# osqp/miosqp

Hardware: AMD Instinct MI355X
Metric: ADMM iterations/s (random_miqp n=500 m=1000 p=250, node-at-a-time B&B) (higher is better)
Workload: dtype f64

## Files before the change

### include/miosqp_amd.h

```cpp
#ifndef MIOSQP_AMD_H
#define MIOSQP_AMD_H

#include <stdint.h>

#ifdef __cplusplus
extern "C" {
#endif

#define MIOSQP_QP_SOLVED 1
#define MIOSQP_QP_MAX_ITER_REACHED (-2)
#define MIOSQP_QP_PRIMAL_INFEASIBLE (-3)
#define MIOSQP_QP_DUAL_INFEASIBLE (-4)
#define MIOSQP_QP_UNSOLVED (-10)

#define MIOSQP_EARG (-1)
#define MIOSQP_EHIP (-2)
#define MIOSQP_EFACTOR (-3)
#define MIOSQP_ENODEV (-4)
#define MIOSQP_EUNSUPPORTED (-5)
#define MIOSQP_EFULL (-6)
#define MIOSQP_EBOUNDS 1

typedef struct miosqp_qp_settings {
  double rho;
// ... 288 lines not shown
  int32_t improved;
  int32_t reserved;
  double upper_glob, lower_glob;
  double device_time;
  double run_time;
} miosqp_search_info;

int miosqp_qp_search_create(miosqp_qp_engine *e, int32_t capacity);
int miosqp_qp_search_reset(miosqp_qp_engine *e);
int miosqp_qp_search_add_leaf(miosqp_qp_engine *e, const double *l_int, const double *u_int, const double *x0,
                              const double *y0, int32_t depth, double lower);
int miosqp_qp_search_take_leaf(miosqp_qp_engine *e, double *l_int, double *u_int, double *x0, double *y0,
                               int32_t *depth, double *lower);
int miosqp_qp_search_set_incumbent(miosqp_qp_engine *e, double upper, const double *x);
int miosqp_qp_search_get_incumbent(miosqp_qp_engine *e, double *upper, double *x);
int miosqp_qp_search_run(miosqp_qp_engine *e, int32_t tree_explor_rule, int64_t max_nodes, double budget_s,
                         miosqp_search_info *info);

typedef struct miosqp_pool_digest {
  int32_t slot;
  int32_t status_val;
  int32_t iter;
  int32_t int_inf;
  int32_t nextvar;
  int32_t reserved;
  double lower;
  double heur_viol;
  double heur_obj;
  double pri_res, dua_res;
} miosqp_pool_digest;
// ... 74 lines not shown
```

### miosqp_amd/_lib.py

```python
import ctypes as C
import os

_PKG = os.path.dirname(os.path.abspath(__file__))
LIB_PATH = os.path.join(_PKG, "libmiosqp_hip.so")

dp = C.POINTER(C.c_double)
ip = C.POINTER(C.c_int32)
i64p = C.POINTER(C.c_int64)


class Settings(C.Structure):
    _fields_ = [(k, C.c_double) for k in
                ("rho", "sigma", "alpha", "eps_abs", "eps_rel", "eps_prim_inf", "eps_dual_inf")] + \
               [(k, C.c_int32) for k in ("max_iter", "scaling", "check_termination", "warm_start",
                                         "device", "max_batch", "fold", "resident", "setup_on_device", "coop", "pers", "batch_pers",
                                         "rho_auto")]


class Info(C.Structure):
    _fields_ = [("status_val", C.c_int32), ("iter", C.c_int32), ("run_time", C.c_double),
                ("obj_val", C.c_double), ("pri_res", C.c_double), ("dua_res", C.c_double),
                ("device_time", C.c_double), ("lower", C.c_double),
                ("int_inf", C.c_int32), ("nextvar", C.c_int32), ("heur_viol", C.c_double),
                ("heur_obj", C.c_double)]
# ... 115 lines not shown
    "miosqp_qp_solve_trees_lockstep_sb": (C.c_int, [C.c_void_p, C.c_int32, dp, dp, dp, dp, dp, dp, dp, C.c_int32, C.c_int32,
                                                    C.c_int32, C.c_int32, C.c_int32, C.c_int32, C.c_int32, C.c_double, dp,
                                                    C.POINTER(TreeInfo), C.POINTER(LockstepStats),
                                                    C.POINTER(LockstepSbStats)]),
    "miosqp_qp_solve_trees_lockstep_ahead": (C.c_int, [C.c_void_p, C.c_int32, dp, dp, dp, dp, dp, dp, dp, C.c_int32,
                                                       C.c_int32, C.c_int32, C.c_int32, dp, C.POINTER(TreeInfo),
                                                       C.POINTER(LockstepStats), C.POINTER(LockstepAheadStats)]),
    "miosqp_qp_solve_trees_refill": (C.c_int, [C.c_void_p, C.c_int32, dp, dp, dp, dp, dp, dp, dp, C.c_int32, C.c_int32,
                                               C.c_int32, dp, C.POINTER(TreeInfo), C.POINTER(RefillStats)]),
    "miosqp_qp_search_create": (C.c_int, [C.c_void_p, C.c_int32]),
    "miosqp_qp_search_reset": (C.c_int, [C.c_void_p]),
    "miosqp_qp_search_add_leaf": (C.c_int, [C.c_void_p, dp, dp, dp, dp, C.c_int32, C.c_double]),
    "miosqp_qp_search_take_leaf": (C.c_int, [C.c_void_p, dp, dp, dp, dp, C.POINTER(C.c_int32), C.POINTER(C.c_double)]),
    "miosqp_qp_search_set_incumbent": (C.c_int, [C.c_void_p, C.c_double, dp]),
    "miosqp_qp_search_get_incumbent": (C.c_int, [C.c_void_p, C.POINTER(C.c_double), dp]),
    "miosqp_qp_search_run": (C.c_int, [C.c_void_p, C.c_int32, C.c_int64, C.c_double, C.POINTER(SearchInfo)]),
    "miosqp_qp_stream_create": (C.c_int, [C.c_void_p, C.c_int32, C.c_int32, C.c_int32]),
    "miosqp_qp_stream_begin": (C.c_int, [C.c_void_p]),
    "miosqp_qp_stream_add_leaf": (C.c_int, [C.c_void_p, dp, dp, dp, dp, C.c_int32, C.c_double]),
    "miosqp_qp_stream_take_leaf": (C.c_int, [C.c_void_p, dp, dp, dp, dp, C.POINTER(C.c_int32), C.POINTER(C.c_double)]),
    "miosqp_qp_stream_set_incumbent": (C.c_int, [C.c_void_p, C.c_double, dp]),
    "miosqp_qp_stream_get_incumbent": (C.c_int, [C.c_void_p, C.POINTER(C.c_double), dp]),
    "miosqp_qp_stream_step": (C.c_int, [C.c_void_p, C.c_int32, C.c_int32, C.c_int32, C.c_int64, C.POINTER(StreamInfo)]),
    "miosqp_qp_solve_batch": (C.c_int, [C.c_void_p, C.c_int32, dp, dp, dp, dp, dp, dp,
                                        C.POINTER(Info)]),
    "miosqp_qp_solve_batch_q": (C.c_int, [C.c_void_p, C.c_int32, dp, dp, dp, dp, dp, dp, dp,
                                          C.POINTER(Info)]),
    "miosqp_qp_solve_tree": (C.c_int, [C.c_void_p, dp, dp, dp, dp, C.c_double, dp, C.c_int32, C.c_int32, dp,
                                       C.POINTER(TreeInfo)]),
    "miosqp_qp_pool_create": (C.c_int, [C.c_void_p, C.c_int32, C.c_int32]),
# ... 70 lines not shown
```

### miosqp_amd/csrc/engine.hip

```cpp
#include <hip/hip_runtime.h>

#include <dlfcn.h>
#include <sys/stat.h>

#include <algorithm>
#include <chrono>
#include <cmath>
#include <cstdio>
#include <cstdlib>
#include <cstring>
#include <map>
#include <mutex>
#include <queue>
#include <deque>
#include <tuple>
#include <type_traits>
#include <string>
#include <vector>

#include "../../include/miosqp_amd.h"
#include "factor.hpp"
#include "polish_many.hpp"
#include "polish_many_large.hpp"
#include "lockstep_trees.hpp"
// ... 77 lines not shown
  int digest;
  int bm_ablate;
  unsigned long long *prof;
  const double *W;
  int ldw;
  unsigned *coop_tag;
  unsigned long long *coop_buf;
  unsigned long long *coop_chk;
  unsigned long long *coop_q;
  unsigned long long *coop_reg;
  unsigned long long *coop_chz;
  unsigned long long *coop_dec;
  int coop_nt;
  int coop_lag;
  int coop_tres;
  const double *Kc;
  int coop_dbg;
  int coop_nap;
  int coop_stride;
  size_t coop_half;
  const double *coop_W;
  int coop_ldw, coop_mg;
  const int *coop_brow;
  const double *coop_aj;
  int Bs;
  double *b_l, *b_u, *b_x, *b_z, *b_y, *b_wh, *b_rx, *b_cv, *b_ut, *b_xt, *b_dx, *b_dy;
  double *b_xfs;
  double *b_sm, *b_sn;
  double *b_xfin, *b_yfin;
  double *b_xi, *b_xis;
// ... 2244 lines not shown
    return pad;
  }
  if (which == 4) {
    ChipTurn *t = chip_of(e);
    if (!t) return -1;
    std::lock_guard<std::mutex> lk(t->mu);
    return t->users;
  }
  if (which == 5) return (e->pers_capable && e->pp.sinv && e->pp.res_w) ? e->n - e->pp.res_c0 : 0;
  if (which == 6) return (e->pers_capable && e->pp.sinv && e->pp.sym) ? e->pp.sym_tiles : 0;
  if (which == 7) return e->kbs_launches;
  if (which == 8) return e->kbs_chunks_run;
  if (which == 9) return e->graph_chunks_run;
  if (which == 10) return e->run_nap_in_use;
  if (which == 11) return e->run_cal_nodes;
  if (which == 12) return e->polml ? (int64_t)(e->polml->cap_slab * sizeof(double)) : 0;
  return which == 0 ? e->compactions : which == 1 ? e->kbp_fallbacks : -1;
}

int miosqp_qp_get_batch_stats(miosqp_qp_engine *e, double *ms, int64_t *batch_iters, int64_t *node_iters,
                              int32_t reset) {
  if (!e) return MIOSQP_EARG;
  if (ms) *ms = e->bloop_ms;
  if (batch_iters) *batch_iters = e->bloop_iters;
  if (node_iters) *node_iters = e->bloop_node_iters;
  if (reset) {
    e->bloop_ms = 0.0;
    e->bloop_iters = e->bloop_node_iters = 0;
  }
  return 0;
// ... 86 lines not shown
```

### miosqp_amd/csrc/host.inc

```
constexpr int POOL_EVENTS = 8;
constexpr int COOP_RETRY = -1000;

inline int pick_tpr(double avg_row) {
  if (avg_row <= 48) return 16;
  if (avg_row <= 192) return 32;
  if (avg_row <= 640) return 64;
  if (avg_row <= 1536) return 128;
  return 256;
}

#define DISPATCH_TPR(tpr, KERNEL, rows, stream, ...)                                              \
  do {                                                                                            \
    switch (tpr) {                                                                                \
      case 16: hipLaunchKernelGGL(KERNEL<16>, dim3(((rows) + 15) / 16), dim3(256), 0, stream, __VA_ARGS__); break;   \
      case 32: hipLaunchKernelGGL(KERNEL<32>, dim3(((rows) + 7) / 8), dim3(256), 0, stream, __VA_ARGS__); break;     \
      case 64: hipLaunchKernelGGL(KERNEL<64>, dim3(((rows) + 3) / 4), dim3(256), 0, stream, __VA_ARGS__); break;     \
      case 128: hipLaunchKernelGGL(KERNEL<128>, dim3(((rows) + 1) / 2), dim3(256), 0, stream, __VA_ARGS__); break;   \
      default: hipLaunchKernelGGL(KERNEL<256>, dim3(rows), dim3(256), 0, stream, __VA_ARGS__); break;                \
    }                                                                                             \
  } while (0)

std::mutex g_capture_mutex;

struct ParkedChunk {
// ... 411 lines not shown
  return 8;
}
int coop_pick_testers(int spare) {
  int nt = spare >= 8 ? std::min(COOP_NT_MAX, spare) : 0;
  if (const char *ev = getenv("MIOSQP_COOP_TESTERS")) nt = std::max(0, std::min(std::min(COOP_NT_MAX, spare), atoi(ev)));
  return nt;
}
void coop_pick_lag(miosqp_qp_engine *e) {
  Dev &d = e->d;
  const int n = e->n, M = e->M, N = n + M, nt = d.coop_nt;
  bool res = nt > 0 && (N % 2) == 0 && N - (M & ~1) <= 128 * COOP_RC_S && M <= COOP_RC_R * nt * 8 && n <= COOP_RV_R * nt * 8 &&
             N <= 128 * COOP_RV_S;
  if (const char *ev = getenv("MIOSQP_COOP_TRES")) res = res && atoi(ev) != 0;
  d.coop_tres = res ? 1 : 0;
  d.coop_lag = res ? 10 : 16;
  if (const char *ev = getenv("MIOSQP_COOP_LAG")) d.coop_lag = std::max(1, atoi(ev));
}

#define COOP_FORMS(X) \
  X(8, 2, 2) X(8, 2, 4) X(8, 3, 4) X(8, 4, 4)
int coop_occupancy(int rw, int cpt, int cptf) {
  int per_cu = 0;
  hipError_t oq = hipErrorInvalidValue;
#define X(RW, CPT, CPTF) \
  if (rw == RW && cpt == CPT && cptf == CPTF) oq = hipOccupancyMaxActiveBlocksPerMultiprocessor(&per_cu, k_coop<512, RW, CPT, CPTF, true>, 512, 0);
  COOP_FORMS(X)
#undef X
  return oq == hipSuccess ? per_cu : 0;
}

// ... 1155 lines not shown
```

### miosqp_amd/csrc/host_search.inc

```
namespace {

struct NodeSearch {
  int cap = 0;
  double *lo = nullptr, *hi = nullptr, *x = nullptr, *y = nullptr, *inc_x = nullptr;
  double *own_block = nullptr;
  SearchDigest *dg = nullptr;
  unsigned long long seq = 0;
  hipEvent_t ev[4] = {};
  int ev_slot = 0;
  bool ev_pending = false;
  unsigned long long *stamps = nullptr;
  std::vector<int> stamp_iter;
  CoopRun *run_blk = nullptr;
  CoopRun run_blk_host;
  bool run_blk_sent = false;
  unsigned long long *mail_host = nullptr, *mail_dev = nullptr;
  unsigned long long mtag = 0;
  bool run_live = false;
  hipEvent_t ev_run[2] = {};
  int64_t run_off = 0;
  int run_nap = -1;
  std::vector<int> open;
  std::vector<int> freelist, depth, parent, kids;
  std::vector<char> decided;
// ... 429 lines not shown
  S.upper = upper;
  S.have_inc = true;
  search_prune(S);
  return 0;
}

int miosqp_qp_search_get_incumbent(miosqp_qp_engine *e, double *upper, double *x) {
  if (!e || !e->search || !upper || !x) return MIOSQP_EARG;
  ENTER(e);
  NodeSearch &S = *search_of(e);
  *upper = S.upper;
  if (S.have_inc) {
    HIPCHK(hipMemcpyAsync(x, S.inc_x, sizeof(double) * e->n, hipMemcpyDeviceToHost, e->stream));
    HIPCHK(hipStreamSynchronize(e->stream));
  }
  return 0;
}

int miosqp_qp_search_run(miosqp_qp_engine *e, int32_t tree_explor_rule, int64_t max_nodes, double budget_s,
                         miosqp_search_info *info) {
  if (!e || !e->search || !info || tree_explor_rule < 0 || tree_explor_rule > 3) return MIOSQP_EARG;
  ENTER(e);
  NodeSearch &S = *search_of(e);
  const double t0 = wall();
  const size_t n = e->n, M = e->M, p = e->d.n_int;
  const Dev &d = e->d;
  int64_t done = 0, it_sum = 0;
  int improved = 0, rc_full = 0;
  double dev_ms = 0.0;
  if (int rc = run_end(e, S, true, nullptr, nullptr)) return rc;
// ... 157 lines not shown
      if (!g.pad) break;
      reset_registration(e);
      g_err = "cooperative solver: " + std::string(g.pad == 1 ? "the grid was not co-resident within 100 ms (device shared?)"
                                                               : "exchange timed out") + ", stage " + std::to_string(g.pad);
      if (g.pad != 1) return MIOSQP_EHIP;
      if (S.ev_pending) {
        HIPCHK(hipEventSynchronize(S.ev[2 * S.ev_slot + 1]));
        S.ev_pending = false;
      }
      e->loop_iters -= g.iter;
      if (!e->node_it.empty()) e->node_it.pop_back();
      int rc = leave_coop(e);
      if (rc) return rc;
    }
    if (S.stamps) S.stamp_iter[a.seq % 256] = g.todo ? -1 : g.iter;
    done++;
    S.nodes++;
    S.iters += g.iter;
    it_sum += g.iter;
    bool branch = false;
    const bool ok = g.status == MIOSQP_QP_SOLVED || g.status == MIOSQP_QP_MAX_ITER_REACHED;
    if (ok) {
      S.lower[s] = g.lower;
      if (!(g.lower > S.upper)) {
        if (g.int_inf == 0) {
          S.upper = g.lower;
          S.have_inc = true;
          improved = 1;
          search_prune(S);
        } else {
// ... 75 lines not shown
```

### miosqp_amd/csrc/kernels_coop.inc

```
constexpr unsigned long long COOP_LIMIT_REGISTER = 10000000ull, COOP_LIMIT_EXCHANGE = 200000000ull;
__device__ __forceinline__ bool coop_expired(unsigned &spins, unsigned long long &since,
                                             unsigned long long limit = COOP_LIMIT_EXCHANGE) {
  if ((++spins & 4095u) != 0u) return false;
  const unsigned long long now = wall_clock64();
  if (spins == 4096u) {
    since = now;
    return false;
  }
  return now - since > limit;
}

typedef unsigned ll_u4 __attribute__((ext_vector_type(4)));
__device__ __forceinline__ void ll_publish(unsigned long long *slot, double v, unsigned tag) {
  ll_u4 w;
  w.x = (unsigned)__double2loint(v); w.y = tag; w.z = (unsigned)__double2hiint(v); w.w = tag;
  asm volatile("global_store_dwordx4 %0, %1, off sc1\n\ts_nop 1" ::"v"(slot), "v"(w) : "memory");
}
__device__ __forceinline__ ll_u4 ll_peek(const unsigned long long *slot) {
  ll_u4 w;
  asm volatile("global_load_dwordx4 %0, %1, off sc1" : "=v"(w) : "v"(slot) : "memory");
  return w;
}

constexpr unsigned long long COOP_SENTINEL = 0x7FF0000000005EA7ull;
// ... 393 lines not shown
  return v;
}

struct CoopTesterArgs {
  unsigned long long *coop_chk, *coop_chz, *coop_q, *coop_dec, *prof;
  const double *Kc, *Einv, *E, *Dinv, *D, *l, *u, *q;
  Ctrl *ctrl;
  int n, M, ldw;
  double c, cinv, eps_abs, eps_rel, eps_pinf, eps_dinf;
  int epi;
  unsigned long long *stamps;
  int res;
  int run;
  unsigned long long *coop_buf, coop_half;
  int NR, lag;
};
#define COOP_STAMP(ptr, k)                                          \
  do {                                                              \
    if ((ptr) != nullptr && threadIdx.x == 0) (ptr)[k] = wall_clock64(); \
  } while (0)

__device__ __forceinline__ double coop_prow(const int *__restrict__ idx, const double *__restrict__ val, int s, int e, int t, int tpr,
                                            const lds_f64 *v) {
  double a0 = 0.0, a1 = 0.0;
  for (int k = s + 2 * t; k < e; k += 2 * tpr) {
    const double2 a = *reinterpret_cast<const double2 *>(val + k);
    const int2 j = *reinterpret_cast<const int2 *>(idx + k);
    a0 = fma(a.x, v[j.x], a0);
    a1 = fma(a.y, v[j.y], a1);
  }
  return a0 + a1;
// ... 86 lines not shown
  const CoopEpi &d = *dp;
  const int t = threadIdx.x, n = d.n, M = d.M;
  lds_f64 *const ox = to_lds(s1), *const xi = to_lds(s1) + 1024, *const xis = to_lds(s2);
  const lds_f64 *const lx = to_lds(lv0);
  for (int i = t; i < n; i += COOP_B) {
    double o = d.D[i] * lx[M + i];
    const int k = d.int_pos[i];
    if (k >= 0) o = fmin(fmax(o, epi_ld(d.a.lo_s + k, d.coh)), epi_ld(d.a.hi_s + k, d.coh));
    ox[i] = o;
    const double r = k >= 0 ? rint(o) : o;
    xi[i] = r;
    xis[i] = d.Dinv[i] * r;
  }
  __syncthreads();
  COOP_STAMP(stamps, 11);
  double vmax = -1.7e308;
  const int Gh = COOP_B / d.tpr_h, Go = COOP_B / d.tpr_o;
  const int CH = (M + Gh - 1) / Gh, CO = (n + Go - 1) / Go;
  for (int c = w; c < CH + CO; c += G) {
    if (c < CH) {
      const int tpr = d.tpr_h, g = t / tpr, tr = t % tpr;
      const int row_raw = c * Gh + g;
      const bool live = row_raw < M;
      const int row = live ? row_raw : M - 1;
      const double ei = d.Einv[row], rl = d.root_l[row], ru = d.root_u[row];
      double acc[1];
      acc[0] = coop_prow(d.pc_idx, d.pc_A, d.pc_ptr[row], d.pc_ptr[row + 1], tr, tpr, xis);
      coop_row_reduce<1>(acc, tpr, red);
      if (live && tr == 0) {
        const double z = ei * acc[0];
// ... 17 lines not shown
  COOP_STAMP(stamps, 12);
  {
    for (int off = 32; off > 0; off >>= 1) vmax = fmax(vmax, __shfl_xor(vmax, off, 64));
    __syncthreads();
    if ((t & 63) == 0) red[t >> 6] = vmax;
    __syncthreads();
    if (t == 0) {
      double r = red[0];
      for (int k = 1; k < COOP_B / 64; k++) r = fmax(r, red[k]);
      ll_publish(d.epi_buf + 2 * (size_t)(2 * n + w), r, tag);
    }
    __syncthreads();
  }
}
template <int COOP_B>
__device__ __attribute__((noinline)) void coop_epi_commit(const CoopEpi *dp, unsigned long long *stamps, const int G, const unsigned tag,
                                                const int st, const int it, const double *lv0, double *s1, double *s2, double *red,
                                                const double *rec, int *s_fail) {
  const CoopEpi &d = *dp;
  const int t = threadIdx.x, n = d.n, M = d.M, p = d.n_int;
  lds_f64 *const ox = to_lds(s1), *const xi = to_lds(s1) + 1024;
  lds_f64 *const vals = to_lds(s2);
  const lds_f64 *const ly = to_lds(lv0);
  COOP_STAMP(stamps, 8);
  int cnt = 0, bestk = 0x7fffffff;
  double best = -1.0;
  for (int k = t; k < p; k += COOP_B) {
    const double v = ox[d.i_idx[k]], f = fabs(v - rint(v));
    cnt += f > d.eps_int;
    if (f > best) { best = f; bestk = k; }
  }
  for (int off = 32; off > 0; off >>= 1) {
    const double ob = __shfl_xor(best, off, 64);
// ... 3 lines not shown
  }
  __shared__ double sb[COOP_B / 64];
  __shared__ int sk[COOP_B / 64], sc[COOP_B / 64], s_dig[2];
  if ((t & 63) == 0) { sb[t >> 6] = best; sk[t >> 6] = bestk; sc[t >> 6] = cnt; }
  __syncthreads();
  if (t == 0) {
    for (int k = 1; k < COOP_B / 64; k++) {
      cnt += sc[k];
      if (sb[k] > best || (sb[k] == best && sk[k] < bestk)) { best = sb[k]; bestk = sk[k]; }
    }
    s_dig[0] = cnt;
    s_dig[1] = bestk == 0x7fffffff ? -1 : bestk;
  }
  __syncthreads();
  const int int_inf = s_dig[0], nv = s_dig[1];
  for (int i = t; i < n; i += COOP_B) epi_st(d.a.x_s + i, ox[i], d.coh);
  for (int r = t; r < M; r += COOP_B) epi_st(d.a.y_s + r, d.cinv * d.E[r] * ly[r], d.coh);
  {
    const int ne = 2 * n + G;
    constexpr int KE = (COOP_EPI_ENTRIES + COOP_B - 1) / COOP_B;
    bool have[KE];
#pragma unroll
    for (int k = 0; k < KE; k++) have[k] = t + k * COOP_B >= ne;
    unsigned spins = 0;
    unsigned long long since = 0;
    static_assert(KE == 5, "ll_peek_wait5");
    for (;;) {
      const unsigned long long *ptr[KE];
      ll_u4 w[KE];
#pragma unroll
      for (int k = 0; k < KE; k++) ptr[k] = d.epi_buf + (have[k] ? 0 : 2 * (size_t)(t + k * COOP_B));
      ll_peek_wait5(ptr, w);
      bool all = true;
#pragma unroll
      for (int k = 0; k < KE; k++) {
        if (have[k]) continue;
        if (w[k].y == tag && w[k].w == tag) {
          vals[t + k * COOP_B] = __hiloint2double((int)w[k].z, (int)w[k].x);
          have[k] = true;
        } else {
          all = false;
        }
      }
      if (__syncthreads_and(all)) break;
      if (coop_expired(spins, since)) {
        *s_fail = 1;
        d.ctrl->pad = 12;
      }
      if (__syncthreads_or(*s_fail)) break;
    }
  }
  __syncthreads();
  if (*s_fail) return;
  COOP_STAMP(stamps, 9);
  const double lower = coop_block_sum1024(vals, n, red);
  const double hobj = coop_block_sum1024(vals + n, n, red);
  __syncthreads();
  double hviol = -1.7e308;
  for (int k = t; k < G; k += COOP_B) hviol = fmax(hviol, vals[2 * n + k]);
  for (int off = 32; off > 0; off >>= 1) hviol = fmax(hviol, __shfl_xor(hviol, off, 64));
  if ((t & 63) == 0) red[t >> 6] = hviol;
  __syncthreads();
  hviol = red[0];
  for (int k = 1; k < COOP_B / 64; k++) hviol = fmax(hviol, red[k]);
  __syncthreads();
  COOP_STAMP(stamps, 14);
  int action = 0, branched = 0;
  if (!(lower > d.a.upper)) {
    if (int_inf == 0) {
      action = 1;
    } else {
      if (hviol <= 0.0 && hobj < d.a.upper) action = 2;
      if (nv >= 0) {
        branched = 1;
        const double xv = ox[d.i_idx[nv]];
        for (int q = t; q < p; q += COOP_B) {
          const double lo = epi_ld(d.a.lo_s + q, d.coh), hi = epi_ld(d.a.hi_s + q, d.coh);
          epi_st(d.a.lo0 + q, lo, d.coh);
          epi_st(d.a.hi0 + q, q == nv ? floor(xv) : hi, d.coh);
          epi_st(d.a.lo1 + q, q == nv ? ceil(xv) : lo, d.coh);
          epi_st(d.a.hi1 + q, hi, d.coh);
        }
      }
    }
  }
  if (action) {
    const lds_f64 *src = action == 1 ? ox : xi;
    for (int i = t; i < n; i += COOP_B) epi_st(d.a.inc_x + i, src[i], d.coh);
  }
  if (d.coh) {
    asm volatile("s_waitcnt vmcnt(0)" ::: "memory");
    __syncthreads();
  }
  COOP_STAMP(stamps, 15);
  if (t == 0) {
    Ctrl *c = d.ctrl;
    c->status = st;
    c->done = 1;
    c->int_inf = int_inf;
    c->nextvar = nv;
    c->lower = lower;
    c->heur_obj = hobj;
    c->heur_viol = hviol;
    const lds_f64 *const rc = to_lds(rec);
    coop_record(d.a.dg, st, it, int_inf, nv, action, branched, lower, hviol, hobj, rc[0], rc[1], rc[2], d.t_node, d.a.seq);
    COOP_STAMP(stamps, 10);
  }
}

constexpr int COOP_RC_R = 3, COOP_RC_S = 4, COOP_RV_R = 1, COOP_RV_S = 16;
template <int COOP_B, int CPTF, bool RES>
__device__ __attribute__((noinline)) void coop_tester(const CoopTesterArgs *dp, const CoopEpi *ep, const int T, const int max_iter,
                                            const int check_every, const int final_check, const unsigned base, int *s_fail,
                                            double *lvp, double *lz) {
  CoopTesterArgs d;
  {
    const auto *l = (const __attribute__((address_space(3))) CoopTesterArgs *)dp;
    d.coop_chk = coop_uni(l->coop_chk); d.coop_chz = coop_uni(l->coop_chz); d.coop_q = coop_uni(l->coop_q);
    d.coop_dec = coop_uni(l->coop_dec); d.prof = coop_uni(l->prof); d.Kc = coop_uni(l->Kc); d.Einv = coop_uni(l->Einv);
    d.E = coop_uni(l->E); d.Dinv = coop_uni(l->Dinv); d.D = coop_uni(l->D); d.l = coop_uni(l->l); d.u = coop_uni(l->u);
    d.q = coop_uni(l->q); d.ctrl = coop_uni(l->ctrl); d.n = coop_uni(l->n); d.M = coop_uni(l->M); d.ldw = coop_uni(l->ldw);
    d.c = coop_uni(l->c); d.cinv = coop_uni(l->cinv); d.eps_abs = coop_uni(l->eps_abs); d.eps_rel = coop_uni(l->eps_rel);
    d.eps_pinf = coop_uni(l->eps_pinf); d.eps_dinf = coop_uni(l->eps_dinf); d.epi = coop_uni(l->epi);
    d.stamps = coop_uni(l->stamps); d.res = coop_uni(l->res); d.run = coop_uni(l->run);
    d.coop_buf = coop_uni(l->coop_buf); d.coop_half = coop_uni(l->coop_half); d.NR = coop_uni(l->NR); d.lag = coop_uni(l->lag);
  }
  constexpr int NW = COOP_B / 64;
  lds_f64 *const lv0 = to_lds(lvp), *const lv1 = to_lds(lvp) + 2048, *const lzl = to_lds(lz);
  __shared__ double qw[NW][NQ];
  __shared__ double qall[COOP_NT_MAX * NQ];
  __shared__ double qres[NQ];
  __shared__ int s_status;
  __shared__ double s_rec[3];
  const int t = threadIdx.x, lane = t & 63, wave = t >> 6;
  const int M = d.M, N = d.n + d.M;
  const int j = (int)blockIdx.x - T, NT = (int)gridDim.x - T;
  const double NEUTRAL = -1.7e308;
  const int Ne = N & ~1;
  auto rows_load = [&](auto RC, auto SC, const bool con, const int first, const int step, const int end, auto &a, auto &sc_inv,
                       auto &sc_dir, auto &lo, auto &up, auto &qv) {
// ... 93 lines not shown
#pragma unroll
      for (int i = 0; i < COOP_RC_R; i++) {
        s_rsc[wave][0][i] = rc_si[i]; s_rsc[wave][1][i] = rc_sd[i]; s_rsc[wave][2][i] = rc_lo[i]; s_rsc[wave][3][i] = rc_up[i];
        s_rsc[wave][4][i] = rc_q[i];
      }
#pragma unroll
      for (int i = 0; i < COOP_RV_R; i++) {
        s_rsv[wave][0][i] = rv_si[i]; s_rsv[wave][1][i] = rv_sd[i]; s_rsv[wave][2][i] = rv_lo[i]; s_rsv[wave][3][i] = rv_up[i];
        s_rsv[wave][4][i] = rv_q[i];
      }
    }
    __syncthreads();
  }
  int to_test = check_every > 0 ? check_every : -1;
  bool bounds_fresh = false;
  for (int it = 1; it <= max_iter; it++) {
    bool chk = final_check && it == max_iter;
    if (--to_test == 0) {
      chk = true;
      to_test = check_every;
    }
    if (!chk) continue;
    const unsigned tag = base + 1u + (unsigned)it;
    const bool stamp = d.prof != nullptr && it == 75 && t == 0;
    unsigned long long *const st = d.prof + 8 * blockIdx.x;
    {
      unsigned spins = 0;
      unsigned long long since = 0;
      for (;;) {
        const ll_u4 w = ll_peek_wait(d.coop_chk);
// ... 120 lines not shown
      else batch(integral_constant<int, 2>{}, integral_constant<int, 16>{}, true, fc, step, M);
      if (N <= 1024) batch(integral_constant<int, 4>{}, integral_constant<int, 8>{}, false, fv, step, N);
      else batch(integral_constant<int, 2>{}, integral_constant<int, 16>{}, false, fv, step, N);
      }
    }
    if (lane < NQ) qw[wave][lane] = acc;
    if (stamp) st[2] = wall_clock64();
    __syncthreads();
    if (j == 0) COOP_STAMP(d.stamps, 3);
    if (stamp) st[3] = wall_clock64();
    if (t < NQ) {
      double rq = qw[0][t];
      for (int w = 1; w < NW; w++) rq = t < NQ_MAX ? fmax(rq, qw[w][t]) : rq + qw[w][t];
      ll_publish(d.coop_q + (size_t)j * COOP_QS + 2 * t, rq, tag);
    }
    if (j == 0) {
      {
        constexpr int KC = (COOP_NT_MAX * NQ + COOP_B - 1) / COOP_B;
        const int ne = NT * NQ;
        bool have[KC];
#pragma unroll
        for (int k = 0; k < KC; k++) have[k] = t + k * COOP_B >= ne;
        unsigned spins = 0;
        unsigned long long since = 0;
        static_assert(KC == 3, "ll_peek_waitn<3>");
        for (;;) {
          const unsigned long long *ptr[KC];
          ll_u4 w[KC];
#pragma unroll
          for (int k = 0; k < KC; k++) {
// ... 26 lines not shown
      if (t < NQ) {
        double rq = qall[t];
        for (int m = 1; m < NT; m++) rq = t < NQ_MAX ? fmax(rq, qall[m * NQ + t]) : rq + qall[m * NQ + t];
        qres[t] = rq;
      }
      __syncthreads();
      if (t == 0) {
        Norms nm{qres[0], qres[1], qres[2], qres[3], qres[4], -qres[5], qres[6] * d.cinv, qres[7], qres[8], qres[9],
                 qres[10], qres[11], qres[12], qres[13], qres[14], qres[15], qres[16]};
        double obj;
        const int st = decide_status(d, nm, obj);
        {
          const int last_free = final_check ? max_iter - 1 : max_iter;
          const int pick = it + d.lag < last_free ? it + d.lag : (it > last_free ? it : last_free);
          const unsigned ptag = base + 1u + (unsigned)pick;
          ll_publish8(coop_ring_buf(d.coop_buf, ptag) + coop_ring_slot<COOP_B>(d.NR), ((unsigned long long)ptag << 32) | (unsigned)st);
        }
        ll_publish(d.coop_dec, (double)st, tag);
        Ctrl *c = d.ctrl;
        __hip_atomic_store(&c->iter, it, __ATOMIC_RELAXED, __HIP_MEMORY_SCOPE_AGENT);
        __hip_atomic_store(&c->pri_res, nm.pri, __ATOMIC_RELAXED, __HIP_MEMORY_SCOPE_AGENT);
        __hip_atomic_store(&c->dua_res, nm.dua, __ATOMIC_RELAXED, __HIP_MEMORY_SCOPE_AGENT);
        __hip_atomic_store(&c->obj_val, obj, __ATOMIC_RELAXED, __HIP_MEMORY_SCOPE_AGENT);
        if (st) {
          __hip_atomic_store(&c->status, st, __ATOMIC_RELAXED, __HIP_MEMORY_SCOPE_AGENT);
          __hip_atomic_store(&c->done, 1, __ATOMIC_RELAXED, __HIP_MEMORY_SCOPE_AGENT);
        }
        COOP_STAMP(d.stamps, 5);
        s_rec[0] = nm.pri; s_rec[1] = nm.dua; s_rec[2] = obj;
        s_status = st;
      }
      __syncthreads();
    } else {
// ... 13 lines not shown
            break;
          }
          __builtin_amdgcn_s_sleep(4);
        }
      }
      __syncthreads();
    }
    if (stamp) st[4] = wall_clock64();
    if (*s_fail) return;
    {
      const int stn = s_status;
      const bool last = final_check && it == max_iter;
      if (d.epi && (stn == MIOSQP_QP_SOLVED || (stn == 0 && last))) {
        __syncthreads();
        unsigned long long *const stp = j == 0 ? d.stamps : nullptr;
        COOP_STAMP(stp, 13);
        coop_epi_rows<COOP_B>(ep, stp, (int)blockIdx.x, (int)gridDim.x, tag, lvp, lvp + 2048, lz, &qw[0][0]);
        if (j == 0)
          coop_epi_commit<COOP_B>(ep, stp, (int)gridDim.x, tag, stn == 0 ? MIOSQP_QP_MAX_ITER_REACHED : stn, it, lvp, lvp + 2048, lz,
                                  &qw[0][0], s_rec, s_fail);
        return;
      }
      if (d.epi && stn != 0) {
        if (j == 0 && t == 0) {
          Ctrl *c = d.ctrl;
          const double nan = __builtin_nan("");
          c->int_inf = -1;
          c->nextvar = -1;
          c->lower = c->heur_obj = c->heur_viol = nan;
          coop_record(ep->a.dg, stn, it, -1, -1, 0, 0, nan, nan, nan, s_rec[0], s_rec[1], s_rec[2], ep->t_node, ep->a.seq);
          COOP_STAMP(d.stamps, 10);
        }
        return;
      }
    }
// ... 144 lines not shown
}

template <class DV, class NV>
__device__ __forceinline__ void coop_fill_epi(CoopEpi *ep, const DV &d, const NV &nd, const int coh) {
  *ep = CoopEpi{d.D, d.Dinv, d.E, d.Einv, d.pc_A, d.pr_val, d.qraw, d.root_l, d.root_u, d.int_pos, d.i_idx,
                d.pc_ptr, d.pc_idx, d.pr_ptr, d.pr_idx, d.ctrl, d.n, d.M, d.n_int, nd.tpr_h, nd.tpr_o, d.cinv,
                d.eps_int, d.eps_lin, SearchArgs{nd.a.lo_s, nd.a.hi_s, nd.a.x_w, nd.a.y_w, nd.a.x_s, nd.a.y_s, nd.a.lo0, nd.a.hi0,
                                                 nd.a.lo1, nd.a.hi1, nd.a.inc_x, nd.a.upper, nd.a.dg, nd.a.seq},
                nd.epi_buf, nullptr, coh, (unsigned long long)wall_clock64()};
}
template <class DV, class NV>
__device__ __forceinline__ void coop_fill_tester(CoopTesterArgs *ta, const DV &d, const NV &nd, const int run) {
  *ta = CoopTesterArgs{d.coop_chk, d.coop_chz, d.coop_q, d.coop_dec, d.prof, d.Kc, d.Einv, d.E, d.Dinv, d.D, d.l,
                       d.u, d.q, d.ctrl, d.n, d.M, d.ldw, d.c, d.cinv, d.eps_abs, d.eps_rel,
                       d.eps_pinf, d.eps_dinf, nd.on && nd.epi, nd.on ? nd.stamps : nullptr, d.coop_tres, run,
                       d.coop_buf, (unsigned long long)d.coop_half, d.coop_mg + d.n, d.coop_lag};
}
__device__ __forceinline__ void coop_ctrl_reset(Ctrl *c) {
  c->done = 0;
  c->pad = 0;
  c->status = MIOSQP_QP_UNSOLVED;
  c->iter = 0;
  c->pri_res = c->dua_res = c->obj_val = 0.0;
  c->lower = __builtin_nan("");
}

template <int RW, int NW, bool TST>
struct CoopLds {
  __attribute__((aligned(16))) double part[2][RW][NW];
  double s_ko[RW][6];
  __attribute__((aligned(16))) double lvs[TST ? 2 * 2048 : 2];
// ... 337 lines not shown

    const long long k0 = prof ? clock64() : 0;
    {
      const CoopTest ta{d.coop_chk, d.coop_q, d.Kc, d.Einv, d.E, d.Dinv, d.D, d.coop_aj, d.ctrl, d.n, d.M, mg, d.ldw,
                        d.c, d.cinv, d.eps_abs, d.eps_rel, d.eps_pinf, d.eps_dinf};
      status = coop_test<COOP_B, RW, CPTF>(ta, tag, it, own, o, &s_fail);
    }
    if (prof) {
      ph3 += clock64() - k0;
      nchk++;
    }
    if (s_fail) break;
    if (status) break;
    }
  }
  if constexpr (TST) {
    if (!called_off) {
      if (it > max_iter) __syncthreads();
      const int dv = s_fail ? 0 : s_dec;
      if (dv) {
        status = dv;
        if (own) { o.z = s_ko[t][0]; o.y = s_ko[t][1]; o.dy = s_ko[t][2]; o.sw = s_ko[t][3]; o.x = s_ko[t][4]; o.dx = s_ko[t][5]; }
        it_rep = last;
      }
    }
  }
  GRID_STAMP(6);
  if (it > max_iter) it = max_iter;
  const int it_done = it;
  if (it_rep >= 0) it = it_rep;
  if (prof && t == 0) {
    unsigned long long *out = d.prof + 8 * blockIdx.x;
    out[0] = ph0; out[1] = ph1; out[2] = ph2; out[3] = it; out[4] = ph3; out[5] = ph4; out[6] = nchk; out[7] = ph5;
  }
  if (own && !called_off) {
    if (con) { d.z[o.rowc] = o.z; d.y[o.rowc] = o.y; d.dy[o.rowc] = o.dy; d.wh[o.rowc] = o.sw; }
    if (var) { d.x[o.var] = o.x; d.dx[o.var] = o.dx; d.rx[o.var] = sigma * o.x - o.q; }
  }
  GRID_STAMP(7);
  const bool epi_here = TST && nd.on && nd.epi && !called_off && !s_fail &&
                        (status == MIOSQP_QP_SOLVED || (status == 0 && final_check && it_rep < 0));
  const bool rec_here = epi_here || (TST && nd.on && nd.epi && !called_off && !s_fail && status != 0);
  if constexpr (TST) {
    if (epi_here) {
      if (t == 0) fill_epi();
      const unsigned etag = base + 1u + (unsigned)it;
      const int n = d.n;
      for (int i0 = 0; i0 < n; i0 += COOP_B) {
        const int i = i0 + t;
        const unsigned long long *ptr = d.coop_chk + 4 * (size_t)(M + (i < n ? i : 0));
        unsigned spins = 0;
        unsigned long long since = 0;
        for (;;) {
          const ll_u4 w = ll_peek_wait(ptr);
          if (w.y == etag && w.w == etag) {
            if (i < n) lvs[M + i] = __hiloint2double((int)w.z, (int)w.x);
            break;
// ... 154 lines not shown
```

### miosqp_amd/qp.py

```python
import ctypes as C
import types

import numpy as np
import scipy.sparse as spa

from miosqp_amd import _lib

_ALIASES = {"eps_inf": "eps_prim_inf", "eps_unb": "eps_dual_inf",
            "early_terminate_interval": "check_termination"}
_IGNORED = {"verbose", "polish", "polishing", "linsys_solver", "time_limit", "scaled_termination",
            "delta", "polish_refine_iter", "early_terminate"}


def constant(name):
    v = _lib.load().miosqp_qp_constant(name.encode())
    if v == 0:
        raise ValueError("Constant %s not found" % name)
    return v


def default_settings():
    s = _lib.Settings()
    _lib.load().miosqp_qp_default_settings(C.byref(s))
    return s
# ... 552 lines not shown
        rc = _check(self._lib.miosqp_qp_search_take_leaf(self._h, _vec(l, n_int, "l_int"), _vec(u, n_int, "u_int"),
                                                         _vec(x, self.n, "x0"), _vec(y, self.m, "y0"),
                                                         C.byref(depth), C.byref(lower)), "search_take_leaf")
        return None if rc == 1 else (l, u, x, y, depth.value, lower.value)

    def search_set_incumbent(self, upper, x):
        _check(self._lib.miosqp_qp_search_set_incumbent(self._h, float(upper),
                                                        None if x is None else _lib.as_d(_f64(x, self.n, "x"))),
               "search_set_incumbent")

    def search_get_incumbent(self):
        upper, x = C.c_double(), np.empty(self.n)
        _check(self._lib.miosqp_qp_search_get_incumbent(self._h, C.byref(upper), _lib.as_d(x)), "search_get_incumbent")
        return (upper.value, x) if upper.value < 1.7e308 else (float("inf"), None)

    def search_run(self, tree_explor_rule, max_nodes, budget_s=0.0):
        info = self._search_info
        max_nodes = 2 ** 62 if not np.isfinite(max_nodes) else int(min(int(max_nodes), 2 ** 62))
        rc = self._lib.miosqp_qp_search_run(self._h, int(tree_explor_rule), max_nodes, float(budget_s), C.byref(info))
        info.full = rc == -6
        if not info.full:
            _check(rc, "search_run")
        return info

    def stream_create(self, capacity, columns, ring_margin=0):
        _check(self._lib.miosqp_qp_stream_create(self._h, int(capacity), int(columns), int(ring_margin)), "stream_create")
        self._stream_info = _lib.StreamInfo()

    def stream_begin(self):
        _check(self._lib.miosqp_qp_stream_begin(self._h), "stream_begin")
# ... 136 lines not shown
        v, k = np.zeros(3), C.c_int32()
        _check(self._lib.miosqp_qp_get_node_stats(self._h, _lib.as_d(v), C.byref(k)), "get_node_stats")
        return float(v[0]), float(v[1]), float(v[2]), k.value

    def loop_launches(self):
        k = C.c_int64()
        _check(self._lib.miosqp_qp_get_loop_launches(self._h, C.byref(k)), "get_loop_launches")
        return k.value

    def batch_stats(self, reset=False):
        ms, bi, ni = C.c_double(), C.c_int64(), C.c_int64()
        _check(self._lib.miosqp_qp_get_batch_stats(self._h, C.byref(ms), C.byref(bi), C.byref(ni), int(reset)),
               "get_batch_stats")
        return ms.value, bi.value, ni.value

    def compactions(self):
        return int(self._lib.miosqp_qp_debug_counter(self._h, 0))

    def batch_pers_fallbacks(self):
        return int(self._lib.miosqp_qp_debug_counter(self._h, 1))

    def stream_chunks_by_form(self):
        return tuple(int(self._lib.miosqp_qp_debug_counter(self._h, k)) for k in (7, 8, 9))

    def resident_grid_poll_delay(self):
        return int(self._lib.miosqp_qp_debug_counter(self._h, 10)), int(self._lib.miosqp_qp_debug_counter(self._h, 11))

    def chip_turn_waits(self):
        return int(self._lib.miosqp_qp_debug_counter(self._h, 2))

# ... 32 lines not shown
```

Baseline: 591,900.

## Run node epilogue speculatively on cooperative tester blocks before the decision

When resident testers are enabled with at least nine tester blocks, the non-leader tester blocks compute the node epilogue (lower bound, heuristic rows, digest) in parallel with the convergence decision. The last tester commits it only after reading the published status and residuals. Grid blocks that see a spec-flagged decision skip their own epilogue. The aim is to take the per-node epilogue off the critical path, at the cost of extra tester work, stale-tag detection, and more complex synchronisation. Debug helpers for inspecting the last node and the tester configuration are added too.

```diff
diff --git a/include/miosqp_amd.h b/include/miosqp_amd.h
--- a/include/miosqp_amd.h
+++ b/include/miosqp_amd.h
@@ -326,6 +326,7 @@
                                int32_t *depth, double *lower);
 int miosqp_qp_search_set_incumbent(miosqp_qp_engine *e, double upper, const double *x);
 int miosqp_qp_search_get_incumbent(miosqp_qp_engine *e, double *upper, double *x);
+int miosqp_qp_search_last_node(miosqp_qp_engine *e, double *rec, double *x, double *y, double *kids);
 int miosqp_qp_search_run(miosqp_qp_engine *e, int32_t tree_explor_rule, int64_t max_nodes, double budget_s,
                          miosqp_search_info *info);
 
diff --git a/miosqp_amd/_lib.py b/miosqp_amd/_lib.py
--- a/miosqp_amd/_lib.py
+++ b/miosqp_amd/_lib.py
@@ -153,6 +153,7 @@
     "miosqp_qp_search_take_leaf": (C.c_int, [C.c_void_p, dp, dp, dp, dp, C.POINTER(C.c_int32), C.POINTER(C.c_double)]),
     "miosqp_qp_search_set_incumbent": (C.c_int, [C.c_void_p, C.c_double, dp]),
     "miosqp_qp_search_get_incumbent": (C.c_int, [C.c_void_p, C.POINTER(C.c_double), dp]),
+    "miosqp_qp_search_last_node": (C.c_int, [C.c_void_p, dp, dp, dp, dp]),
     "miosqp_qp_search_run": (C.c_int, [C.c_void_p, C.c_int32, C.c_int64, C.c_double, C.POINTER(SearchInfo)]),
     "miosqp_qp_stream_create": (C.c_int, [C.c_void_p, C.c_int32, C.c_int32, C.c_int32]),
     "miosqp_qp_stream_begin": (C.c_int, [C.c_void_p]),
diff --git a/miosqp_amd/csrc/engine.hip b/miosqp_amd/csrc/engine.hip
--- a/miosqp_amd/csrc/engine.hip
+++ b/miosqp_amd/csrc/engine.hip
@@ -115,6 +115,7 @@
   int coop_nt;
   int coop_lag;
   int coop_tres;
+  int coop_espec;
   const double *Kc;
   int coop_dbg;
   int coop_nap;
@@ -2389,6 +2390,15 @@
   if (which == 9) return e->graph_chunks_run;
   if (which == 10) return e->run_nap_in_use;
   if (which == 11) return e->run_cal_nodes;
+  if (which == 13) {
+    if (e->device >= 0 && hipSetDevice(e->device) != hipSuccess) return -1;
+    int k = -1;
+    if (hipStreamSynchronize(e->stream) != hipSuccess) return -1;
+    if (hipMemcpy(&k, &e->d.ctrl->pad4[0], sizeof k, hipMemcpyDeviceToHost) != hipSuccess) return -1;
+    return k;
+  }
+  if (which == 14) return e->coop ? e->d.coop_nt : 0;
+  if (which == 15) return e->coop ? (e->d.coop_tres | (e->d.coop_espec << 1)) : 0;
   if (which == 12) return e->polml ? (int64_t)(e->polml->cap_slab * sizeof(double)) : 0;
   return which == 0 ? e->compactions : which == 1 ? e->kbp_fallbacks : -1;
 }
diff --git a/miosqp_amd/csrc/host.inc b/miosqp_amd/csrc/host.inc
--- a/miosqp_amd/csrc/host.inc
+++ b/miosqp_amd/csrc/host.inc
@@ -449,6 +449,10 @@
   if (const char *ev = getenv("MIOSQP_COOP_TRES")) res = res && atoi(ev) != 0;
   d.coop_tres = res ? 1 : 0;
   d.coop_lag = res ? 10 : 16;
+  {
+    const char *ev = getenv("MIOSQP_COOP_EPI_SPEC");
+    d.coop_espec = (res && nt >= 9 && !(ev && atoi(ev) == 0)) ? 1 : 0;
+  }
   if (const char *ev = getenv("MIOSQP_COOP_LAG")) d.coop_lag = std::max(1, atoi(ev));
 }
 
diff --git a/miosqp_amd/csrc/host_search.inc b/miosqp_amd/csrc/host_search.inc
--- a/miosqp_amd/csrc/host_search.inc
+++ b/miosqp_amd/csrc/host_search.inc
@@ -6,6 +6,8 @@
   double *own_block = nullptr;
   SearchDigest *dg = nullptr;
   unsigned long long seq = 0;
+  SearchDigest last_g{};
+  int last_s = -1, last_c0 = -1, last_c1 = -1;
   hipEvent_t ev[4] = {};
   int ev_slot = 0;
   bool ev_pending = false;
@@ -467,6 +469,27 @@
     HIPCHK(hipMemcpyAsync(x, S.inc_x, sizeof(double) * e->n, hipMemcpyDeviceToHost, e->stream));
     HIPCHK(hipStreamSynchronize(e->stream));
   }
+  return 0;
+}
+
+int miosqp_qp_search_last_node(miosqp_qp_engine *e, double *rec, double *x, double *y, double *kids) {
+  if (!e || !e->search || !rec || !x || !y || !kids) return MIOSQP_EARG;
+  ENTER(e);
+  NodeSearch &S = *search_of(e);
+  if (S.last_s < 0) return 1;
+  const SearchDigest &g = S.last_g;
+  const double r[12] = {(double)g.status, (double)g.iter, (double)g.int_inf, (double)g.nextvar, (double)g.action, (double)g.branched,
+                        g.lower, g.heur_viol, g.heur_obj, g.pri_res, g.dua_res, g.obj_val};
+  memcpy(rec, r, sizeof r);
+  const size_t n = e->n, M = e->M, p = e->d.n_int;
+  HIPCHK(hipMemcpyAsync(x, S.x + S.last_s * n, sizeof(double) * n, hipMemcpyDeviceToHost, e->stream));
+  HIPCHK(hipMemcpyAsync(y, S.y + S.last_s * M, sizeof(double) * M, hipMemcpyDeviceToHost, e->stream));
+  const int c[2] = {S.last_c0, S.last_c1};
+  for (int k = 0; k < 2; k++) {
+    HIPCHK(hipMemcpyAsync(kids + (2 * k) * p, S.lo + c[k] * p, sizeof(double) * p, hipMemcpyDeviceToHost, e->stream));
+    HIPCHK(hipMemcpyAsync(kids + (2 * k + 1) * p, S.hi + c[k] * p, sizeof(double) * p, hipMemcpyDeviceToHost, e->stream));
+  }
+  HIPCHK(hipStreamSynchronize(e->stream));
   return 0;
 }
 
@@ -654,6 +677,8 @@
       if (rc) return rc;
     }
     if (S.stamps) S.stamp_iter[a.seq % 256] = g.todo ? -1 : g.iter;
+    S.last_g = g;
+    S.last_s = s; S.last_c0 = c0; S.last_c1 = c1;
     done++;
     S.nodes++;
     S.iters += g.iter;
diff --git a/miosqp_amd/csrc/kernels_coop.inc b/miosqp_amd/csrc/kernels_coop.inc
--- a/miosqp_amd/csrc/kernels_coop.inc
+++ b/miosqp_amd/csrc/kernels_coop.inc
@@ -431,7 +431,10 @@
   int run;
   unsigned long long *coop_buf, coop_half;
   int NR, lag;
+  int spec;
 };
+constexpr int COOP_DEC_SPEC = 0x20000000;
+__device__ __forceinline__ bool coop_dec_spec(int dv) { return (dv & 0x60000000) == COOP_DEC_SPEC; }
 #define COOP_STAMP(ptr, k)                                          \
   do {                                                              \
     if ((ptr) != nullptr && threadIdx.x == 0) (ptr)[k] = wall_clock64(); \
@@ -548,6 +551,10 @@
   }
   __syncthreads();
   COOP_STAMP(stamps, 11);
+  if (w < 0) {
+    COOP_STAMP(stamps, 12);
+    return;
+  }
   double vmax = -1.7e308;
   const int Gh = COOP_B / d.tpr_h, Go = COOP_B / d.tpr_o;
   const int CH = (M + Gh - 1) / Gh, CO = (n + Go - 1) / Go;
@@ -595,9 +602,9 @@
   }
 }
 template <int COOP_B>
-__device__ __attribute__((noinline)) void coop_epi_commit(const CoopEpi *dp, unsigned long long *stamps, const int G, const unsigned tag,
-                                                const int st, const int it, const double *lv0, double *s1, double *s2, double *red,
-                                                const double *rec, int *s_fail) {
+__device__ __attribute__((noinline)) int coop_epi_commit(const CoopEpi *dp, unsigned long long *stamps, const int G, const unsigned tag,
+                                               const int st_in, const int it, const double *lv0, double *s1, double *s2, double *red,
+                                               double *rec, int *s_fail, const unsigned long long *dec, const int last) {
   const CoopEpi &d = *dp;
   const int t = threadIdx.x, n = d.n, M = d.M, p = d.n_int;
   lds_f64 *const ox = to_lds(s1), *const xi = to_lds(s1) + 1024;
@@ -631,8 +638,15 @@
   }
   __syncthreads();
   const int int_inf = s_dig[0], nv = s_dig[1];
-  for (int i = t; i < n; i += COOP_B) epi_st(d.a.x_s + i, ox[i], d.coh);
-  for (int r = t; r < M; r += COOP_B) epi_st(d.a.y_s + r, d.cinv * d.E[r] * ly[r], d.coh);
+  lds_f64 *const lyw = to_lds(const_cast<double *>(lv0));
+  if (dec != nullptr)
+    for (int r = t; r < M; r += COOP_B) lyw[r] = d.cinv * d.E[r] * ly[r];
+  auto slot = [&]() {
+    for (int i = t; i < n; i += COOP_B) epi_st(d.a.x_s + i, ox[i], d.coh);
+    for (int r = t; r < M; r += COOP_B) epi_st(d.a.y_s + r, dec != nullptr ? ly[r] : d.cinv * d.E[r] * ly[r], d.coh);
+  };
+  if (dec == nullptr) slot();
+  bool stale = false;
   {
     const int ne = 2 * n + G;
     constexpr int KE = (COOP_EPI_ENTRIES + COOP_B - 1) / COOP_B;
@@ -657,6 +671,7 @@
           have[k] = true;
         } else {
           all = false;
+          if (dec != nullptr && w[k].y == w[k].w && (int)(w[k].y - tag) > 0) stale = true;
         }
       }
       if (__syncthreads_and(all)) break;
@@ -664,11 +679,11 @@
         *s_fail = 1;
         d.ctrl->pad = 12;
       }
-      if (__syncthreads_or(*s_fail)) break;
-    }
-  }
-  __syncthreads();
-  if (*s_fail) return;
+      if (__syncthreads_or(*s_fail | (int)stale)) break;
+    }
+  }
+  if (__syncthreads_or((int)stale)) return 0;
+  if (*s_fail) return 0;
   COOP_STAMP(stamps, 9);
   const double lower = coop_block_sum1024(vals, n, red);
   const double hobj = coop_block_sum1024(vals + n, n, red);
@@ -682,6 +697,35 @@
   for (int k = 1; k < COOP_B / 64; k++) hviol = fmax(hviol, red[k]);
   __syncthreads();
   COOP_STAMP(stamps, 14);
+  int st = st_in;
+  if (dec != nullptr) {
+    __shared__ double s_dv[4];
+    if (t < 4) {
+      unsigned spins = 0;
+      unsigned long long since = 0;
+      for (;;) {
+        const ll_u4 w = ll_peek_wait(dec + 2 * t);
+        if (w.y == tag && w.w == tag) {
+          s_dv[t] = __hiloint2double((int)w.z, (int)w.x);
+          break;
+        }
+        if (*s_fail) break;
+        if (coop_expired(spins, since)) {
+          *s_fail = 1;
+          d.ctrl->pad = 14;
+          break;
+        }
+      }
+    }
+    __syncthreads();
+    if (*s_fail) return 0;
+    const int sd = (int)s_dv[0];
+    if (!(sd == MIOSQP_QP_SOLVED || (sd == 0 && last))) return 0;
+    st = sd == 0 ? MIOSQP_QP_MAX_ITER_REACHED : sd;
+    if (t == 0) { rec[0] = s_dv[1]; rec[1] = s_dv[2]; rec[2] = s_dv[3]; }
+    COOP_STAMP(stamps, 13);
+    slot();
+  }
   int action = 0, branched = 0;
   if (!(lower > d.a.upper)) {
     if (int_inf == 0) {
@@ -712,17 +756,15 @@
   COOP_STAMP(stamps, 15);
   if (t == 0) {
     Ctrl *c = d.ctrl;
-    c->status = st;
-    c->done = 1;
-    c->int_inf = int_inf;
-    c->nextvar = nv;
-    c->lower = lower;
-    c->heur_obj = hobj;
-    c->heur_viol = hviol;
+#define CTRL_ST(f, v) __hip_atomic_store(&c->f, v, __ATOMIC_RELAXED, __HIP_MEMORY_SCOPE_AGENT)
+    CTRL_ST(status, st); CTRL_ST(done, 1); CTRL_ST(int_inf, int_inf); CTRL_ST(nextvar, nv);
+    CTRL_ST(lower, lower); CTRL_ST(heur_obj, hobj); CTRL_ST(heur_viol, hviol);
+#undef CTRL_ST
     const lds_f64 *const rc = to_lds(rec);
     coop_record(d.a.dg, st, it, int_inf, nv, action, branched, lower, hviol, hobj, rc[0], rc[1], rc[2], d.t_node, d.a.seq);
     COOP_STAMP(stamps, 10);
   }
+  return 1;
 }
 
 constexpr int COOP_RC_R = 3, COOP_RC_S = 4, COOP_RV_R = 1, COOP_RV_S = 16;
@@ -741,6 +783,7 @@
     d.eps_pinf = coop_uni(l->eps_pinf); d.eps_dinf = coop_uni(l->eps_dinf); d.epi = coop_uni(l->epi);
     d.stamps = coop_uni(l->stamps); d.res = coop_uni(l->res); d.run = coop_uni(l->run);
     d.coop_buf = coop_uni(l->coop_buf); d.coop_half = coop_uni(l->coop_half); d.NR = coop_uni(l->NR); d.lag = coop_uni(l->lag);
+    d.spec = coop_uni(l->spec);
   }
   constexpr int NW = COOP_B / 64;
   lds_f64 *const lv0 = to_lds(lvp), *const lv1 = to_lds(lvp) + 2048, *const lzl = to_lds(lz);
@@ -864,6 +907,7 @@
   }
   int to_test = check_every > 0 ? check_every : -1;
   bool bounds_fresh = false;
+  const bool spec = RES && d.spec != 0 && NT > 2;
   for (int it = 1; it <= max_iter; it++) {
     bool chk = final_check && it == max_iter;
     if (--to_test == 0) {
@@ -1014,6 +1058,17 @@
       for (int w = 1; w < NW; w++) rq = t < NQ_MAX ? fmax(rq, qw[w][t]) : rq + qw[w][t];
       ll_publish(d.coop_q + (size_t)j * COOP_QS + 2 * t, rq, tag);
     }
+    if (spec && j != 0) {
+      if (j < NT - 1) {
+        coop_epi_rows<COOP_B>(ep, j == 1 ? d.stamps : nullptr, j - 1, NT - 2, tag, lvp, lvp + 2048, lz, &qw[0][0]);
+      } else {
+        coop_epi_rows<COOP_B>(ep, nullptr, -1, NT - 2, tag, lvp, lvp + 2048, lz, &qw[0][0]);
+        const int wrote = coop_epi_commit<COOP_B>(ep, d.stamps, NT - 2, tag, 0, it, lvp, lvp + 2048, lz, &qw[0][0], s_rec, s_fail,
+                                                  d.coop_dec, final_check && it == max_iter);
+        if (wrote && t == 0) __hip_atomic_fetch_add(&d.ctrl->pad4[0], 1, __ATOMIC_RELAXED, __HIP_MEMORY_SCOPE_AGENT);
+        if (*s_fail) return;
+      }
+    }
     if (j == 0) {
       {
         constexpr int KC = (COOP_NT_MAX * NQ + COOP_B - 1) / COOP_B;
@@ -1070,9 +1125,16 @@
           const int last_free = final_check ? max_iter - 1 : max_iter;
           const int pick = it + d.lag < last_free ? it + d.lag : (it > last_free ? it : last_free);
           const unsigned ptag = base + 1u + (unsigned)pick;
-          ll_publish8(coop_ring_buf(d.coop_buf, ptag) + coop_ring_slot<COOP_B>(d.NR), ((unsigned long long)ptag << 32) | (unsigned)st);
+          const bool sol = st == MIOSQP_QP_SOLVED || (st == 0 && final_check && it == max_iter);
+          const unsigned stw = (unsigned)st | (spec && sol ? (unsigned)COOP_DEC_SPEC : 0u);
+          ll_publish8(coop_ring_buf(d.coop_buf, ptag) + coop_ring_slot<COOP_B>(d.NR), ((unsigned long long)ptag << 32) | stw);
         }
         ll_publish(d.coop_dec, (double)st, tag);
+        if (spec) {
+          ll_publish(d.coop_dec + 2, nm.pri, tag);
+          ll_publish(d.coop_dec + 4, nm.dua, tag);
+          ll_publish(d.coop_dec + 6, obj, tag);
+        }
         Ctrl *c = d.ctrl;
         __hip_atomic_store(&c->iter, it, __ATOMIC_RELAXED, __HIP_MEMORY_SCOPE_AGENT);
         __hip_atomic_store(&c->pri_res, nm.pri, __ATOMIC_RELAXED, __HIP_MEMORY_SCOPE_AGENT);
@@ -1116,11 +1178,12 @@
       if (d.epi && (stn == MIOSQP_QP_SOLVED || (stn == 0 && last))) {
         __syncthreads();
         unsigned long long *const stp = j == 0 ? d.stamps : nullptr;
+        if (spec) return;
         COOP_STAMP(stp, 13);
         coop_epi_rows<COOP_B>(ep, stp, (int)blockIdx.x, (int)gridDim.x, tag, lvp, lvp + 2048, lz, &qw[0][0]);
         if (j == 0)
           coop_epi_commit<COOP_B>(ep, stp, (int)gridDim.x, tag, stn == 0 ? MIOSQP_QP_MAX_ITER_REACHED : stn, it, lvp, lvp + 2048, lz,
-                                  &qw[0][0], s_rec, s_fail);
+                                  &qw[0][0], s_rec, s_fail, nullptr, 0);
         return;
       }
       if (d.epi && stn != 0) {
@@ -1295,7 +1358,8 @@
   *ta = CoopTesterArgs{d.coop_chk, d.coop_chz, d.coop_q, d.coop_dec, d.prof, d.Kc, d.Einv, d.E, d.Dinv, d.D, d.l,
                        d.u, d.q, d.ctrl, d.n, d.M, d.ldw, d.c, d.cinv, d.eps_abs, d.eps_rel,
                        d.eps_pinf, d.eps_dinf, nd.on && nd.epi, nd.on ? nd.stamps : nullptr, d.coop_tres, run,
-                       d.coop_buf, (unsigned long long)d.coop_half, d.coop_mg + d.n, d.coop_lag};
+                       d.coop_buf, (unsigned long long)d.coop_half, d.coop_mg + d.n, d.coop_lag,
+                       nd.on && nd.epi && d.coop_tres && d.coop_espec};
 }
 __device__ __forceinline__ void coop_ctrl_reset(Ctrl *c) {
   c->done = 0;
@@ -1663,10 +1727,13 @@
     if (status) break;
     }
   }
+  bool epi_spec = false;
   if constexpr (TST) {
     if (!called_off) {
       if (it > max_iter) __syncthreads();
-      const int dv = s_fail ? 0 : s_dec;
+      const int dw = s_fail ? 0 : s_dec;
+      epi_spec = coop_dec_spec(dw);
+      const int dv = epi_spec ? dw & ~COOP_DEC_SPEC : dw;
       if (dv) {
         status = dv;
         if (own) { o.z = s_ko[t][0]; o.y = s_ko[t][1]; o.dy = s_ko[t][2]; o.sw = s_ko[t][3]; o.x = s_ko[t][4]; o.dx = s_ko[t][5]; }
@@ -1687,9 +1754,9 @@
     if (var) { d.x[o.var] = o.x; d.dx[o.var] = o.dx; d.rx[o.var] = sigma * o.x - o.q; }
   }
   GRID_STAMP(7);
-  const bool epi_here = TST && nd.on && nd.epi && !called_off && !s_fail &&
+  const bool epi_here = TST && nd.on && nd.epi && !called_off && !s_fail && !epi_spec &&
                         (status == MIOSQP_QP_SOLVED || (status == 0 && final_check && it_rep < 0));
-  const bool rec_here = epi_here || (TST && nd.on && nd.epi && !called_off && !s_fail && status != 0);
+  const bool rec_here = epi_here || epi_spec || (TST && nd.on && nd.epi && !called_off && !s_fail && status != 0);
   if constexpr (TST) {
     if (epi_here) {
       if (t == 0) fill_epi();
diff --git a/miosqp_amd/qp.py b/miosqp_amd/qp.py
--- a/miosqp_amd/qp.py
+++ b/miosqp_amd/qp.py
@@ -590,6 +590,18 @@
         _check(self._lib.miosqp_qp_search_get_incumbent(self._h, C.byref(upper), _lib.as_d(x)), "search_get_incumbent")
         return (upper.value, x) if upper.value < 1.7e308 else (float("inf"), None)
 
+    def search_last_node(self, n_int):
+        rec, x, y, kids = np.empty(12), np.empty(self.n), np.empty(self.m), np.empty(4 * n_int)
+        rc = _check(self._lib.miosqp_qp_search_last_node(self._h, _lib.as_d(rec), _lib.as_d(x), _lib.as_d(y), _lib.as_d(kids)),
+                    "search_last_node")
+        if rc == 1:
+            return None
+        names = ("status", "iter", "int_inf", "nextvar", "action", "branched")
+        out = {k: int(rec[i]) for i, k in enumerate(names)}
+        out.update(lower=rec[6], heur_viol=rec[7], heur_obj=rec[8], pri_res=rec[9], dua_res=rec[10], obj_val=rec[11],
+                   x=x, y=y, kids=kids.reshape(4, n_int))
+        return out
+
     def search_run(self, tree_explor_rule, max_nodes, budget_s=0.0):
         info = self._search_info
         max_nodes = 2 ** 62 if not np.isfinite(max_nodes) else int(min(int(max_nodes), 2 ** 62))
@@ -756,6 +768,10 @@
                "get_batch_stats")
         return ms.value, bi.value, ni.value
 
+    def coop_testers(self):
+        k = [int(self._lib.miosqp_qp_debug_counter(self._h, w)) for w in (13, 14, 15)]
+        return dict(testers=k[1], resident_rows=bool(k[2] & 1), speculative_epilogue=bool(k[2] & 2), commits=k[0])
+
     def compactions(self):
         return int(self._lib.miosqp_qp_debug_counter(self._h, 0))
 
```

After: 581,300. -1.8%, worse.
